# fetty31/fast_LIMO

Hardware: AMD Instinct MI355X
Metric: scans/sec (64k-pt scan, 1M-pt map) + kNN HBM GB/s vs roofline; ATE vs CPU ref (higher is better)
Workload: dtype f32; 1 GPU; BASELINE.json configs[1]: 65536-pt Velodyne-like scan (64 rings x 1024 azimuths), 1000000-pt box-world map, k=5, MAX_NUM_ITERS=3, GPU deskew + iterated ESKF update per step; parallelism=replicas x1 (independent scan streams, no collective), steps_bit_reproducible=True, chains_run=0, chains_handed_back_early=0, chains_declined=2597

## Files before the change

fast_limo_amd/csrc/hip/flimo_kernels.hip:

```cpp
#include <hip/hip_runtime.h>
#include <hip/hip_ext.h>
#include <float.h>
#include <limits.h>
#include <stdlib.h>
#include <algorithm>
#include "flimo_types.h"
#include "flimo_math.h"
#include "flimo_kernels.h"
#include "flimo_chain.h"
#include "flimo_ieskf.h"

#pragma clang fp contract(off)

namespace flimo {

FLIMO_DEV bool pair_less(float d0, int i0, float d1, int i1) { return (d0 < d1) || (d0 == d1 && i0 < i1); }

template <int K>
FLIMO_DEV void topk_insert(float (&bd)[K], int (&bi)[K], float d, int id) {
  if (!pair_less(d, id, bd[K - 1], bi[K - 1])) return;
  bd[K - 1] = d;
  bi[K - 1] = id;
#pragma unroll
  for (int s = K - 1; s > 0; s--) {
// ... 32 lines not shown
FLIMO_DEV void merge_group(float (&bd)[K], int (&bi)[K]) {
#pragma unroll
  for (int off = 1; off < L; off <<= 1) {
    float od[K];
    int oi[K];
#pragma unroll
    for (int s = 0; s < K; s++) {
      od[s] = __shfl_xor(bd[s], off, 64);
      oi[s] = __shfl_xor(bi[s], off, 64);
    }
#pragma unroll
    for (int s = 0; s < K; s++) topk_insert<K>(bd, bi, od[s], oi[s]);
  }
}

FLIMO_DEV float slab_dist(int d, float r) {
  return d == 0 ? 0.f : (d > 0 ? ((float)d - r) : (r + (float)(-d - 1)));
}

template <int K = 5>
struct KnnResultK {
  float bd[K];
  int bi[K];
  int cand;
  bool exact;
};
typedef KnnResultK<5> KnnResult;

template <int L, int K>
FLIMO_DEV void visit_row(const GridView& G, int cx, int cy, int cz, int dy, int dz, int r_prev, int r, float rx,
                         float ry, float rz, float margin, float cell2, float bound, int sub, float gx, float gy,
                         float gz, KnnResultK<K>& R) {
  const float a = fmaxf(slab_dist(dy, ry) - margin, 0.f), b = fmaxf(slab_dist(dz, rz) - margin, 0.f);
  const float yz2 = a * a + b * b;
  if (yz2 * cell2 >= fminf(bound, R.bd[K - 1])) return;
  if (max(abs(dy), abs(dz)) > r_prev) {
    const int x0 = max(cx - r, 0), x1 = min(cx + r, G.nx - 1);
    if (x0 <= x1) {
      uint32_t lo, hi;
      grid_row_range(G, G.dir, cy + dy, cz + dz, x0 * G.xs, (x1 + 1) * G.xs, lo, hi);
      scan_range<L, K>(G.pts, lo, hi, sub, gx, gy, gz, R.bd, R.bi, R.cand);
    }
  } else {
    {
      const int x0 = max(cx - r, 0), x1 = min(cx - r_prev - 1, G.nx - 1);
      const float sx = fmaxf(slab_dist(-(r_prev + 1), rx) - margin, 0.f);
      if (x0 <= x1 && (sx * sx + yz2) * cell2 < fminf(bound, R.bd[K - 1])) {
        uint32_t lo, hi;
        grid_row_range(G, G.dir, cy + dy, cz + dz, x0 * G.xs, (x1 + 1) * G.xs, lo, hi);
        scan_range<L, K>(G.pts, lo, hi, sub, gx, gy, gz, R.bd, R.bi, R.cand);
      }
    }
    {
      const int x0 = max(cx + r_prev + 1, 0), x1 = min(cx + r, G.nx - 1);
      const float sx = fmaxf(slab_dist(r_prev + 1, rx) - margin, 0.f);
      if (x0 <= x1 && (sx * sx + yz2) * cell2 < fminf(bound, R.bd[K - 1])) {
        uint32_t lo, hi;
        grid_row_range(G, G.dir, cy + dy, cz + dz, x0 * G.xs, (x1 + 1) * G.xs, lo, hi);
        scan_range<L, K>(G.pts, lo, hi, sub, gx, gy, gz, R.bd, R.bi, R.cand);
      }
    }
  }
}

template <int L, int K = 5>
FLIMO_DEV void knn_search(const GridView& G, float gx, float gy, float gz, int sub, int max_ring, KnnResultK<K>& R) {
#pragma unroll
  for (int s = 0; s < K; s++) { R.bd[s] = FLT_MAX; R.bi[s] = INT_MAX; }
  R.cand = 0;
  R.exact = false;

  const float fx = (gx - G.ox) * G.inv_cell, fy = (gy - G.oy) * G.inv_cell, fz = (gz - G.oz) * G.inv_cell;
  if (!(fx == fx) || !(fy == fy) || !(fz == fz)) return;
  const float lim = 1.0e9f;
  const float flx = floorf(fminf(fmaxf(fx, -lim), lim));
  const float fly = floorf(fminf(fmaxf(fy, -lim), lim));
  const float flz = floorf(fminf(fmaxf(fz, -lim), lim));
  const int cx = (int)flx - G.six, cy = (int)fly - G.siy, cz = (int)flz - G.siz;
  const float rx = fminf(fmaxf(fx - flx, 0.f), 1.f), ry = fminf(fmaxf(fy - fly, 0.f), 1.f),
              rz = fminf(fmaxf(fz - flz, 0.f), 1.f);

  const int maxdim = grid_maxdim(G);
  const float margin = 1.0e-3f + 4.0e-7f * (float)maxdim;
  const float cell2 = G.cell * G.cell;
  const float edge = fminf(fminf(fminf(rx, 1.f - rx), fminf(ry, 1.f - ry)), fminf(rz, 1.f - rz));

  int r0;
  {
    const int ox_ = cx < 0 ? -cx : (cx >= G.nx ? cx - G.nx + 1 : 0);
    const int oy_ = cy < 0 ? -cy : (cy >= G.ny ? cy - G.ny + 1 : 0);
    const int oz_ = cz < 0 ? -cz : (cz >= G.nz ? cz - G.nz + 1 : 0);
    r0 = max(1, max(ox_, max(oy_, oz_)));
  }
  if (r0 > max_ring) return;

  int r_prev = -1;
  int r = r0;
  float bound = FLT_MAX;
  for (;;) {
    if (r == 1) {
      uint32_t lo[9], hi[9];
      const int x0 = max(cx - 1, 0), x1 = min(cx + 1, G.nx - 1);
#pragma unroll
      for (int t = 0; t < 9; t++) {
        const int dy = (t % 3 == 0) ? 0 : ((t % 3 == 1) ? -1 : 1);
        const int dz = (t / 3 == 0) ? 0 : ((t / 3 == 1) ? -1 : 1);
        const int yy = cy + dy, zz = cz + dz;
        const bool in = (yy >= 0) && (yy < G.ny) && (zz >= 0) && (zz < G.nz) && (x0 <= x1);
        lo[t] = 0u; hi[t] = 0u;
        if (in) grid_row_range(G, G.dir, yy, zz, x0 * G.xs, (x1 + 1) * G.xs, lo[t], hi[t]);
      }
#pragma unroll
      for (int t = 0; t < 9; t++) {
        const int dy = (t % 3 == 0) ? 0 : ((t % 3 == 1) ? -1 : 1);
        const int dz = (t / 3 == 0) ? 0 : ((t / 3 == 1) ? -1 : 1);
        const float a = fmaxf(slab_dist(dy, ry) - margin, 0.f), b = fmaxf(slab_dist(dz, rz) - margin, 0.f);
        if ((a * a + b * b) * cell2 >= R.bd[K - 1]) continue;
        scan_range<L, K>(G.pts, lo[t], hi[t], sub, gx, gy, gz, R.bd, R.bi, R.cand);
      }
    } else {
      const int dz0 = max(-r, -cz), dz1 = min(r, G.nz - 1 - cz);
      const int dy0 = max(-r, -cy), dy1 = min(r, G.ny - 1 - cy);
      for (int dz = dz0; dz <= dz1; dz++)
        for (int dy = dy0; dy <= dy1; dy++)
          visit_row<L, K>(G, cx, cy, cz, dy, dz, r_prev, r, rx, ry, rz, margin, cell2, bound, sub, gx, gy, gz, R);
    }
    if (L > 1) merge_group<L, K>(R.bd, R.bi);
    const float rg = ((float)r + edge - margin) * G.cell;
    const bool have5 = R.bi[K - 1] != INT_MAX;
    const bool covers = (cx - r <= 0) && (cx + r >= G.nx - 1) && (cy - r <= 0) && (cy + r >= G.ny - 1) &&
                        (cz - r <= 0) && (cz + r >= G.nz - 1);
    if (covers || (have5 && R.bd[K - 1] <= rg * rg * (1.f - 1.0e-6f))) { R.exact = true; break; }
    if (r >= max_ring) break;
    int rn = 2 * r;
    if (have5) {
      bound = R.bd[K - 1];
      const float need = fl_sqrt(R.bd[K - 1]) * G.inv_cell * (1.f + 4.0e-6f) - edge + margin;
      rn = max(r + 1, (int)ceilf(fminf(need, 1.0e9f)));
    }
    rn = min(rn, max_ring);
    if (L > 1 && sub != 0) {
#pragma unroll
      for (int s = 0; s < K; s++) { R.bd[s] = FLT_MAX; R.bi[s] = INT_MAX; }
    }
    r_prev = r;
    r = rn;
  }
}

typedef unsigned long long u64;
#define KEY_EMPTY 0xffffffffffffffffull

#ifdef FLIMO_TRACE
__device__ unsigned long long g_trace[2][16384 * 8];
#if FLIMO_TRACE == 2
__shared__ unsigned long long s_trace_lds[2][8];
#define TRACE(k, slot)                                                                                  \
  do {                                                                                                  \
    asm volatile("s_waitcnt vmcnt(0) lgkmcnt(0)" ::: "memory");                                         \
    if (threadIdx.x == 0) s_trace_lds[k][slot] = wall_clock64();                                        \
  } while (0)
#define TRACE_LANE(k, slot, tid)                                                                        \
  do {                                                                                                  \
    if (threadIdx.x == (tid)) {                                                                         \
      asm volatile("s_waitcnt vmcnt(0) lgkmcnt(0)" ::: "memory");                                       \
      s_trace_lds[k][slot] = wall_clock64();                                                            \
    }                                                                                                   \
  } while (0)
#define TRACE_FLUSH()                                                                                   \
  do {                                                                                                  \
    __syncthreads();                                                                                    \
    if (threadIdx.x == 0 && blockIdx.x < 16384)                                                         \
      for (int k_ = 0; k_ < 2; k_++) for (int s_ = 0; s_ < 8; s_++) g_trace[k_][blockIdx.x * 8 + s_] = s_trace_lds[k_][s_]; \
  } while (0)
#else
#define TRACE(k, slot)                                                                                  \
  do {                                                                                                  \
    asm volatile("s_waitcnt vmcnt(0) lgkmcnt(0)" ::: "memory");                                         \
    if (threadIdx.x == 0 && blockIdx.x < 16384) g_trace[k][blockIdx.x * 8 + (slot)] = wall_clock64();  \
  } while (0)
#define TRACE_FLUSH() do {} while (0)
#define TRACE_LANE(k, slot, tid) do {} while (0)
#endif
extern "C" int flimo_trace_read(int k, unsigned long long* out, size_t n) {
  return (int)hipMemcpyFromSymbol(out, HIP_SYMBOL(g_trace), n * sizeof(unsigned long long), (size_t)k * 16384 * 8 * sizeof(unsigned long long),
                                  hipMemcpyDeviceToHost);
}
#else
#define TRACE(k, slot) do {} while (0)
#define TRACE_FLUSH() do {} while (0)
#define TRACE_LANE(k, slot, tid) do {} while (0)
#endif

FLIMO_DEV u64 make_key(float d, uint32_t idx) { return ((u64)__float_as_uint(d) << 32) | (u64)idx; }

FLIMO_DEV void key5_insert(u64 (&k)[5], u64 key) {
  if (key >= k[4]) return;
  k[4] = key;
#pragma unroll
  for (int s = 4; s > 0; s--) {
    const u64 a = k[s - 1], b = k[s];
    const bool sw = b < a;
    k[s - 1] = sw ? b : a;
    k[s] = sw ? a : b;
  }
}

__constant__ int c_stripe = 8;
void set_xcd_stripe(int stripe) { (void)hipMemcpyToSymbol(HIP_SYMBOL(c_stripe), &stripe, sizeof(int)); }

__device__ __forceinline__ int xcd_chunk(int b, int nb) {
  const int x = b & 7, k = b >> 3, per = nb >> 3;
  const int S = c_stripe;
  if (S <= 0 || S >= per) return x * per + k;
  const int full = (per / S) * S;
  if (k >= full) return 8 * full + x * (per - full) + (k - full);
  return ((k / S) * 8 + x) * S + (k % S);
}

struct NbrRec {
  int32_t idx[5];
  int32_t flag;
  int32_t d5_bits;
  int32_t d5_valid;
};

struct U3 { uint32_t a, b, c; };
struct __attribute__((aligned(8))) Seg2 { uint32_t x0, y0, x1, y1; };
__device__ __forceinline__ double key_min(double a, double b) { double r; asm("v_min_f64 %0, %1, %2" : "=v"(r) : "v"(a), "v"(b)); return r; }
__device__ __forceinline__ double key_max(double a, double b) { double r; asm("v_max_f64 %0, %1, %2" : "=v"(r) : "v"(a), "v"(b)); return r; }
__device__ __forceinline__ double key_make(float d, uint32_t id) { return __hiloint2double((int)__float_as_uint(d), (int)id); }
__device__ __forceinline__ void best5_insert(double (&k)[5], double x) {
  double t = x;
#pragma unroll
  for (int i = 0; i < 4; i++) {
    const double lo = key_min(k[i], t);
    t = key_max(k[i], t);
    k[i] = lo;
  }
  k[4] = key_min(k[4], t);
}
__device__ __forceinline__ void best6_insert(double (&k)[6], double x) {
  double t = x;
#pragma unroll
  for (int i = 0; i < 5; i++) {
    const double lo = key_min(k[i], t);
    t = key_max(k[i], t);
    k[i] = lo;
  }
  k[5] = key_min(k[5], t);
}
#define KEY_NONE 0x7f800000ffffffffull

template <int CTRL>
__device__ __forceinline__ double key_dpp(double x) {
  const int lo = __double2loint(x), hi = __double2hiint(x);
  const int l2 = __builtin_amdgcn_update_dpp(lo, lo, CTRL, 0xf, 0xf, false);
  const int h2 = __builtin_amdgcn_update_dpp(hi, hi, CTRL, 0xf, 0xf, false);
  return __hiloint2double(h2, l2);
}
__device__ __forceinline__ double key_group_min(double md, int Gl, int lane) {
  md = key_min(md, key_dpp<0xB1>(md));
  if (Gl >= 4) md = key_min(md, key_dpp<0x4E>(md));
  if (Gl >= 8) md = key_min(md, key_dpp<0x141>(md));
  if (Gl >= 16) md = key_min(md, key_dpp<0x140>(md));
  if (Gl >= 32) {
    const int lo = __double2loint(md), hi = __double2hiint(md);
    const double r0 = __hiloint2double(__builtin_amdgcn_readlane(hi, 0), __builtin_amdgcn_readlane(lo, 0));
    const double r1 = __hiloint2double(__builtin_amdgcn_readlane(hi, 16), __builtin_amdgcn_readlane(lo, 16));
    const double r2 = __hiloint2double(__builtin_amdgcn_readlane(hi, 32), __builtin_amdgcn_readlane(lo, 32));
    const double r3 = __hiloint2double(__builtin_amdgcn_readlane(hi, 48), __builtin_amdgcn_readlane(lo, 48));
    const double a = key_min(r0, r1), b = key_min(r2, r3);
    md = (Gl >= 64) ? key_min(a, b) : (lane < 32 ? a : b);
  }
  return md;
}

__device__ __forceinline__ void key_merge6(const double (&a)[6], const double (&b)[6], double (&c)[6]) {
#pragma unroll
  for (int i = 0; i < 6; i++) c[i] = key_min(a[i], b[5 - i]);
#define FLIMO_CE(i, j) { const double lo_ = key_min(c[i], c[j]); c[j] = key_max(c[i], c[j]); c[i] = lo_; }
  FLIMO_CE(0, 5) FLIMO_CE(1, 3) FLIMO_CE(2, 4)
  FLIMO_CE(1, 2) FLIMO_CE(3, 4)
  FLIMO_CE(0, 3) FLIMO_CE(2, 5)
  FLIMO_CE(0, 1) FLIMO_CE(2, 3) FLIMO_CE(4, 5)
  FLIMO_CE(1, 2) FLIMO_CE(3, 4)
#undef FLIMO_CE
}
__device__ __forceinline__ void key_pair_merge6(const double (&a)[6], double (&c)[6]) {
  double b[6];
#pragma unroll
  for (int i = 0; i < 6; i++) b[i] = key_dpp<0xB1>(a[i]);
  key_merge6(a, b, c);
}

template <int L, int N, bool PAYW = false, int NSEG = 9>
__device__ __forceinline__ void knn5_body(const float4* __restrict__ pts, uint32_t s0, uint32_t total, uint32_t last,
                                          const uint32_t (&off)[NSEG + 1], const uint32_t (&dl)[NSEG], float gx, float gy, float gz,
                                          double (&k5)[6]) {
  float4 pt[N];
  uint32_t id[N];
#pragma unroll
  for (int u = 0; u < N; u++) {
    const uint32_t s = min(s0 + u * L, last);
    uint32_t delta = dl[0];
#pragma unroll
    for (int t = 1; t < NSEG; t++) delta = (s >= off[t]) ? dl[t] : delta;
    id[u] = s + delta;
    pt[u] = pts[id[u]];
  }
  if constexpr (N == 8)
    asm volatile("" : "+v"(pt[0].x), "+v"(pt[0].y), "+v"(pt[0].z), "+v"(pt[1].x), "+v"(pt[1].y), "+v"(pt[1].z),
                      "+v"(pt[2].x), "+v"(pt[2].y), "+v"(pt[2].z), "+v"(pt[3].x), "+v"(pt[3].y), "+v"(pt[3].z),
                      "+v"(pt[4].x), "+v"(pt[4].y), "+v"(pt[4].z), "+v"(pt[5].x), "+v"(pt[5].y), "+v"(pt[5].z),
                      "+v"(pt[6].x), "+v"(pt[6].y), "+v"(pt[6].z), "+v"(pt[7].x), "+v"(pt[7].y), "+v"(pt[7].z));
  else if constexpr (N == 4)
    asm volatile("" : "+v"(pt[0].x), "+v"(pt[0].y), "+v"(pt[0].z), "+v"(pt[1].x), "+v"(pt[1].y), "+v"(pt[1].z),
                      "+v"(pt[2].x), "+v"(pt[2].y), "+v"(pt[2].z), "+v"(pt[3].x), "+v"(pt[3].y), "+v"(pt[3].z));
  else if constexpr (N == 2)
    asm volatile("" : "+v"(pt[0].x), "+v"(pt[0].y), "+v"(pt[0].z), "+v"(pt[1].x), "+v"(pt[1].y), "+v"(pt[1].z));
#pragma unroll
  for (int u = 0; u < N; u++) {
    const bool live = s0 + u * L < total;
    const float d = sqdist3(gx, gy, gz, pt[u].x, pt[u].y, pt[u].z);
    best6_insert(k5, key_make(live ? d : INFINITY, live ? (PAYW ? __float_as_uint(pt[u].w) : id[u]) : 0xffffffffu));
  }
}


struct FitIdx { unsigned char raw[FIT_LIVE_PAD]; };
__device__ __forceinline__ bool key_has_tie(const u64 (&best)[5], u64 sixth) {
  const uint32_t d0 = (uint32_t)(best[0] >> 32), d1 = (uint32_t)(best[1] >> 32), d2 = (uint32_t)(best[2] >> 32),
                 d3 = (uint32_t)(best[3] >> 32), d4 = (uint32_t)(best[4] >> 32), d5 = (uint32_t)(sixth >> 32);
  return (d0 == d1) | (d1 == d2) | (d2 == d3) | (d3 == d4) | (d4 == d5);
}
constexpr int TAIL_MAX_RING = 3;
constexpr int KNN_FAR_RING = 4;
constexpr uint32_t PROBE_MIN_OWN = 6;
struct __align__(16) WaveLds {
  float tile[16 * 65];
  double acc[256];
  int src[64];
  int res[64][8];
};
// ... 758 lines not shown
    if (in_range && sub == 0 && flag == 1 && inside) {
      int4 a, b;
      a.x = (int)(uint32_t)best[0]; a.y = (int)(uint32_t)best[1]; a.z = (int)(uint32_t)best[2]; a.w = (int)(uint32_t)best[3];
      b.x = (int)(uint32_t)best[4]; b.y = 4; b.z = (int)(uint32_t)(best[4] >> 32);
      b.w = (int)(1u | (tie ? 2u : 0u) | ((uint32_t)(fa.seq & 0xffffffull) << 8));
      int4* o = reinterpret_cast<int4*>(&nbr[p]);
      o[0] = a;
      o[1] = b;
      if (tie && tl.list) { const unsigned slot = atomicAdd(tl.count, 1u); if (slot < tl.cap) tl.list[slot] = p; }
    }
    return;
  }
  TRACE(0, 4);
  const bool pend_tail = tail && in_range && flag == 2;
  if (in_range && sub == 0 && !pend_tail) {
    int4 a, b;
    a.x = (int)(uint32_t)best[0]; a.y = (int)(uint32_t)best[1]; a.z = (int)(uint32_t)best[2]; a.w = (int)(uint32_t)best[3];
    b.x = (int)(uint32_t)best[4]; b.y = min(flag, 2); b.z = (int)(uint32_t)(best[4] >> 32); b.w = ((flag == 1) ? 1 : 0) | (tie ? 2 : 0);
    if (tie && !tie_listed && tl.list) { const unsigned slot = atomicAdd(tl.count, 1u); if (slot < tl.cap) tl.list[slot] = p; }
    int4* o = reinterpret_cast<int4*>(&nbr[p]);
    o[0] = a;
    o[1] = b;
    if (flag >= 2) {
      const int slot = atomicAdd(wl_count, 1);
      int4* e = reinterpret_cast<int4*>(wl) + 2 * (size_t)slot;
      e[0] = make_int4(p, __float_as_int(gx), __float_as_int(gy), __float_as_int(gz));
      e[1] = make_int4((int)(uint32_t)(best[4] >> 32), 2, __float_as_int(b2), 0);
    }
  }
  WaveLds& W = s_w[threadIdx.x >> 6];
  if (tail) knn5_tail(G, dir, max_ring, nbr, pend_tail && sub == 0, p, gx, gy, gz, (uint32_t)(best[4] >> 32), b2, W, wl_count, cand_total, FUSE, tl);
  TRACE(0, 5);
  if constexpr (FUSE) {
    const int lane = threadIdx.x & 63;
    float v[16];
#pragma unroll
    for (int i = 0; i < 16; i++) v[i] = 0.f;
    wave_lds_sync();
    int ids[5] = {(int)(uint32_t)best[0], (int)(uint32_t)best[1], (int)(uint32_t)best[2], (int)(uint32_t)best[3], (int)(uint32_t)best[4]};
    int fl = flag;
    bool tied = tie;
    uint32_t d5b = (uint32_t)(best[4] >> 32);
    if (sub == 0 && in_range && pend_tail) {
      const int4* rr = reinterpret_cast<const int4*>(W.res[lane]);
      const int4 a = rr[0], b = rr[1];
      ids[0] = a.x; ids[1] = a.y; ids[2] = a.z; ids[3] = a.w; ids[4] = b.x;
      fl = b.y;
      tied = (b.w & 2) != 0;
      d5b = (uint32_t)b.z;
    }
    if (fa.book.node_c)
      tie_repair_wave(G, fa.book, nbr, sub == 0 && in_range && fl == 1 && tied, p, gx, gy, gz, d5b, ids, *reinterpret_cast<TieLds*>(W.tile));
    TRACE(1, 1);
    if (sub == 0 && in_range) {
      if (fl == 1 && __float_as_uint(sp.w) < (uint32_t)fa.mp.n_queries) fit_row(G, P, fa.mp, ids, gx, gy, gz, v);
    }
    TRACE(1, 3);
    wave_lds_sync();
    fit_reduce_publish<64 / L>(v, sub == 0, lane / L, W.tile, s_w[0].acc, s_w[1].acc, s_w[2].acc, s_w[3].acc, &s_last, fa.idx,
                               fa.partials, fa.granules, fa.ticket, wl_count, fa.seq, tl, (int)blockIdx.x, nb);
  }
  TRACE_FLUSH();
}

template <int L, int SLOTS, bool FUSE, bool FINE = false>
__global__ __launch_bounds__(256) KNN_WPE void knn5_kernel(GridView G, const float4* __restrict__ scan_sorted, int n,
                                                   PoseMats P, int max_ring, NbrRec* __restrict__ nbr,
                                                   int* __restrict__ wl, int* __restrict__ wl_count,
                                                   unsigned long long* __restrict__ cand_total, PrevPass prev, int tail,
                                                   FuseArgs fa) {
  __shared__ __align__(16) uint16_t s_dir[GRID_DIR_MAX];
  const DirRegs dr = grid_dir_fetch(G);
  __shared__ PoseMats s_pose;
  static_assert(sizeof(PoseMats) % 4 == 0 && sizeof(PoseMats) / 4 <= 256, "one word per thread");
  if (threadIdx.x < sizeof(PoseMats) / 4)
    reinterpret_cast<uint32_t*>(&s_pose)[threadIdx.x] = reinterpret_cast<const uint32_t*>(&P)[threadIdx.x];
  knn5_pass<L, SLOTS, FUSE, FINE>(G, s_dir, &dr, scan_sorted, n, s_pose, max_ring, nbr, wl, wl_count, cand_total, prev.RT, prev.valid, prev.probe_min, tail, fa);
}
__device__ __forceinline__ const ChainHead* chain_enter(const ChainHead* __restrict__ H, const PipeHead* __restrict__ pipe, const PrevRT& prt,
                                                        unsigned int wait_epoch, unsigned int end_code) {
  constexpr int NW = (int)(sizeof(ChainHead) / 4);
  __shared__ unsigned int s_head[NW];
  __shared__ int s_go;
  if (pipe != nullptr) {
    const int tid = (int)threadIdx.x;
    if (tid < 64) {
      const unsigned long long t0 = wall_clock64();
      int go = 0;
      unsigned long long gv = 0ull;
      unsigned int* dec = const_cast<unsigned int*>(&pipe->decision);
      const unsigned int v_go = wait_epoch, v_pend = wait_epoch | 0x80000000u, v_no = (wait_epoch & 0x3fffffffu) | 0x80000000u;
      for (int look = 0;; look++) {
        const unsigned int d = __hip_atomic_load(dec, __ATOMIC_RELAXED, __HIP_MEMORY_SCOPE_SYSTEM);
        gv = __hip_atomic_load(&pipe->gran[tid], __ATOMIC_RELAXED, __HIP_MEMORY_SCOPE_SYSTEM);
        const unsigned int e = (unsigned int)(gv >> 32);
        const bool all = __ballot(e == wait_epoch) == ~0ull;
        const unsigned int e0 = (unsigned int)__builtin_amdgcn_readfirstlane((int)e);
        if (d == v_no) break;
        if (d == v_pend) { __builtin_amdgcn_s_sleep(8); continue; }
        if (all) { go = 1; break; }
        if (e0 == end_code) break;
        const unsigned long long waited = wall_clock64() - t0;
        if (blockIdx.x == 0 && d != v_go && waited > (unsigned long long)CH_POLL_MS * 100000ull) {
          if (tid == 0) __hip_atomic_store(dec, v_pend, __ATOMIC_RELAXED, __HIP_MEMORY_SCOPE_SYSTEM);
          asm volatile("s_waitcnt vmcnt(0)" ::: "memory");
          for (int nap = 0; nap < 4; nap++) __builtin_amdgcn_s_sleep(127);
          gv = __hip_atomic_load(&pipe->gran[tid], __ATOMIC_RELAXED, __HIP_MEMORY_SCOPE_SYSTEM);
          go = __ballot((unsigned int)(gv >> 32) == wait_epoch) == ~0ull ? 1 : 0;
          if (tid == 0) __hip_atomic_store(dec, go ? v_go : v_no, __ATOMIC_RELAXED, __HIP_MEMORY_SCOPE_SYSTEM);
          break;
        }
        if (waited > 4ull * (unsigned long long)CH_POLL_MS * 100000ull) break;
        if (look == 0) __builtin_amdgcn_s_sleep(48);
        else __builtin_amdgcn_s_sleep(8);
      }
      if (go && tid < PH_WORDS) s_head[tid < 36 ? (tid / 12) * 16 + tid % 12 : tid + 12] = (unsigned int)gv;
      if (tid == 0) s_go = go;
    } else if (tid < 64 + 12) {
      const int k = tid - 64;
      s_head[(k / 4) * 16 + 12 + k % 4] = __float_as_uint(k % 4 == 3 ? 1.f : 0.f);
    } else if (tid >= 128 && tid < 128 + 16) {
      s_head[offsetof(ChainHead, prev_RT) / 4 + (tid - 128)] = __float_as_uint(prt.v[tid - 128]);
    } else if (tid >= 192 && tid < 192 + NW - (int)(offsetof(ChainHead, status) / 4)) {
      s_head[offsetof(ChainHead, status) / 4 + (tid - 192)] = 0u;
    }
    __syncthreads();
    if (!s_go) return nullptr;
  } else {
    if ((int)threadIdx.x < NW) s_head[threadIdx.x] = reinterpret_cast<const unsigned int*>(H)[threadIdx.x];
    __syncthreads();
  }
  const ChainHead* Lh = reinterpret_cast<const ChainHead*>(s_head);
  return Lh->status != 0 ? nullptr : Lh;
}
template <int L, int SLOTS, bool FUSE, bool FINE = false>
__global__ __launch_bounds__(256) KNN_WPE void knn5_chain_kernel(GridView G, const float4* __restrict__ scan_sorted, int n,
                                                   const ChainHead* __restrict__ H, int max_ring, NbrRec* __restrict__ nbr,
                                                   int* __restrict__ wl, int* __restrict__ wl_count,
                                                   unsigned long long* __restrict__ cand_total, int prev_valid, unsigned probe_min, int tail,
                                                   FuseArgs fa, unsigned int wait_epoch, const PipeHead* __restrict__ pipe, PrevRT prt) {
  __shared__ __align__(16) uint16_t s_dir[GRID_DIR_MAX];
  {
    const DirRegs dr = grid_dir_fetch(G);
    grid_dir_store(s_dir, dr);
  }
  const ChainHead* Lh = chain_enter(H, pipe, prt, wait_epoch, fa.ch.end_code);
  if (!Lh) return;
  knn5_pass<L, SLOTS, FUSE, FINE>(G, s_dir, nullptr, scan_sorted, n, Lh->pose, max_ring, nbr, wl, wl_count, cand_total, Lh->prev_RT, prev_valid, probe_min, tail, fa);
}

__device__ __forceinline__ void widen_body(const GridView& G, int max_ring, NbrRec* __restrict__ nbr,
                                           const int* __restrict__ wl, const int* __restrict__ wl_count,
                                           unsigned long long* __restrict__ cand_total, int first_ring, const TieList& tl,
                                           int blk, int nblk, uint32_t (*s_off)[65], uint32_t (*s_lo)[64]) {
  const int lane = threadIdx.x & 63, wave = threadIdx.x >> 6;
  const int maxdim = grid_maxdim(G);
  const float margin = 1.0e-3f + 4.0e-7f * (float)maxdim;
  int w = blk * 4 + wave;
  const int4* entries = reinterpret_cast<const int4*>(wl);
  int4 e0 = entries[2 * (size_t)w], e1 = entries[2 * (size_t)w + 1];
  const int count = *wl_count;
  for (; w < count; w += nblk * 4) {
    if (w != blk * 4 + wave) { e0 = entries[2 * (size_t)w]; e1 = entries[2 * (size_t)w + 1]; }
    const int p = e0.x;
    const float gx = __int_as_float(e0.y), gy = __int_as_float(e0.z), gz = __int_as_float(e0.w);
    const int hint_bits = e1.x;
    const float fx = (gx - G.ox) * G.inv_cell, fy = (gy - G.oy) * G.inv_cell, fz = (gz - G.oz) * G.inv_cell;
    const float flx = floorf(fminf(fmaxf(fx, -1.0e9f), 1.0e9f)), fly = floorf(fminf(fmaxf(fy, -1.0e9f), 1.0e9f)),
                flz = floorf(fminf(fmaxf(fz, -1.0e9f), 1.0e9f));
    const int cx = (int)flx - G.six, cy = (int)fly - G.siy, cz = (int)flz - G.siz;
    const float rx = fminf(fmaxf(fx - flx, 0.f), 1.f), ry = fminf(fmaxf(fy - fly, 0.f), 1.f),
                rz = fminf(fmaxf(fz - flz, 0.f), 1.f);
    const float edge = fminf(fminf(fminf(rx, 1.f - rx), fminf(ry, 1.f - ry)), fminf(rz, 1.f - rz));
    u64 best[5] = {KEY_NONE, KEY_NONE, KEY_NONE, KEY_NONE, KEY_NONE};
    u64 sixth = KEY_NONE;
    int flag = 0;
    int cand = 0;
    int r = first_ring;
    float bnd2 = __int_as_float(e1.z);
    if (!(bnd2 >= 0.f)) bnd2 = INFINITY;
    {
      const float hint = __int_as_float(hint_bits);
      if (hint >= 0.f && hint < INFINITY) {
        const float need = fl_sqrt(hint) * G.inv_cell * (1.f + 4.0e-6f) - edge + margin;
        r = max(2, (int)ceilf(fminf(need, 1.0e9f)));
        const float rc = (fl_sqrt(hint) * (1.f + 1.0e-5f) + 1.0e-6f) * G.inv_cell;
        bnd2 = fminf(bnd2, rc * rc * (1.f + 1.0e-5f));
      }
      r = min(r, max_ring);
    }
    for (;;) {
      const int side = 2 * r + 1;
      uint32_t lo = 0, len = 0;
      if (lane < side * side) {
        const int dy = (lane % side) - r, dz = (lane / side) - r;
        const int yy = cy + dy, zz = cz + dz;
        const float a_ = fmaxf(slab_dist(dy, ry) - margin, 0.f), b_ = fmaxf(slab_dist(dz, rz) - margin, 0.f);
        const float dyz2 = a_ * a_ + b_ * b_;
        int x0 = max(cx - r, 0), x1 = min(cx + r, G.nx - 1);
        if (bnd2 < 1.0e18f) {
          const float xr = fl_sqrt(fmaxf(bnd2 - dyz2, 0.f)) * (1.f + 1.0e-6f) + margin + 1.0e-4f;
          const int dr = (int)fminf(floorf(fminf(xr + rx, 1.0e6f)), (float)r);
          const int dl = (int)fminf(floorf(fminf(xr + (1.f - rx), 1.0e6f)), (float)r);
          x0 = max(cx - dl, 0); x1 = min(cx + dr, G.nx - 1);
        }
        if (dyz2 <= bnd2 && yy >= 0 && yy < G.ny && zz >= 0 && zz < G.nz && x0 <= x1) {
          uint32_t hi_;
          grid_row_range(G, G.dir, yy, zz, x0 * G.xs, (x1 + 1) * G.xs, lo, hi_);
          len = hi_ - lo;
        }
      }
      uint32_t inc = len;
#pragma unroll
      for (int o = 1; o < 64; o <<= 1) {
        const uint32_t v = __shfl_up(inc, o, 64);
        if (lane >= o) inc += v;
      }
      const uint32_t total = __shfl(inc, 63, 64);
      s_off[wave][lane + 1] = inc;
      if (lane == 0) s_off[wave][0] = 0;
      s_lo[wave][lane] = lo;
      __builtin_amdgcn_wave_barrier();
      const double none = __longlong_as_double((long long)KEY_NONE);
      double k5[6] = {none, none, none, none, none, none};
      const uint32_t last = total - 1u;
      for (uint32_t s0 = (uint32_t)lane; s0 < total; s0 += 4 * 64) {
        float4 q[4];
        uint32_t id[4];
#pragma unroll
        for (int u = 0; u < 4; u++) {
          const uint32_t s = min(s0 + 64u * u, last);
          int a = 0;
#pragma unroll
          for (int step = 32; step >= 1; step >>= 1) a = (s_off[wave][a + step] <= s) ? a + step : a;
          id[u] = s_lo[wave][a] + (s - s_off[wave][a]);
          q[u] = G.pts[id[u]];
        }
        asm volatile("" : "+v"(q[0].x), "+v"(q[0].y), "+v"(q[0].z), "+v"(q[1].x), "+v"(q[1].y), "+v"(q[1].z),
                          "+v"(q[2].x), "+v"(q[2].y), "+v"(q[2].z), "+v"(q[3].x), "+v"(q[3].y), "+v"(q[3].z));
#pragma unroll
        for (int u = 0; u < 4; u++) {
          const bool live = s0 + 64u * u < total;
          const float d = sqdist3(gx, gy, gz, q[u].x, q[u].y, q[u].z);
          best6_insert(k5, key_make(live ? d : INFINITY, live ? id[u] : 0xffffffffu));
        }
      }
      cand += total > (uint32_t)lane ? (int)((total - (uint32_t)lane + 63u) / 64u) : 0;
      __builtin_amdgcn_wave_barrier();
      u64 mine[6];
#pragma unroll
      for (int i = 0; i < 6; i++) mine[i] = (u64)__double_as_longlong(k5[i]);
#pragma unroll
      for (int k = 0; k < 6; k++) {
        const double md = key_group_min(__longlong_as_double((long long)mine[0]), 64, lane);
        const u64 m = (u64)__double_as_longlong(md);
        if (k < 5) best[k] = m; else sixth = m;
        if (mine[0] == m) { mine[0] = mine[1]; mine[1] = mine[2]; mine[2] = mine[3]; mine[3] = mine[4]; mine[4] = mine[5]; mine[5] = KEY_NONE; }
      }
      const float rg = ((float)r + edge - margin) * G.cell;
      const float d5 = __uint_as_float((uint32_t)(best[4] >> 32));
      const bool have5 = d5 < INFINITY;
      const bool covers = (cx - r <= 0) && (cx + r >= G.nx - 1) && (cy - r <= 0) && (cy + r >= G.ny - 1) &&
                          (cz - r <= 0) && (cz + r >= G.nz - 1);
      if (have5 && (covers || d5 <= rg * rg * (1.f - 1.0e-6f))) { flag = 1; break; }
      if (covers || r >= max_ring) { flag = 0; break; }
      int rn = r + 1;
      if (have5) {
        const float need = fl_sqrt(d5) * G.inv_cell * (1.f + 4.0e-6f) - edge + margin;
        rn = max(r + 1, (int)ceilf(fminf(need, 1.0e9f)));
        const float rc = (fl_sqrt(d5) * (1.f + 1.0e-5f) + 1.0e-6f) * G.inv_cell;
        bnd2 = fminf(bnd2, rc * rc * (1.f + 1.0e-5f));
      }
      r = min(rn, max_ring);
    }
    if (cand_total) {
      int c = cand;
#pragma unroll
      for (int o = 1; o < 64; o <<= 1) c += __shfl_xor(c, o, 64);
      if (lane == 0) atomicAdd(cand_total, (unsigned long long)c);
    }
    if (lane == 0) {
      int4 a, b;
      a.x = (int)(uint32_t)best[0]; a.y = (int)(uint32_t)best[1]; a.z = (int)(uint32_t)best[2]; a.w = (int)(uint32_t)best[3];
      const bool tie = flag == 1 && key_has_tie(best, sixth);
      b.x = (int)(uint32_t)best[4]; b.y = flag; b.z = (int)(uint32_t)(best[4] >> 32); b.w = ((flag == 1) ? 1 : 0) | (tie ? 2 : 0);
      int4* o = reinterpret_cast<int4*>(&nbr[p]);
      o[0] = a;
      o[1] = b;
      if (tie && tl.list) { const unsigned slot = atomicAdd(tl.count, 1u); if (slot < tl.cap) tl.list[slot] = p; }
    }
  }
}
__global__ __launch_bounds__(256) void widen_kernel(GridView G, const float4* __restrict__ scan_sorted, PoseMats P,
                                                    int max_ring, NbrRec* __restrict__ nbr, const int* __restrict__ wl,
                                                    const int* __restrict__ wl_count,
                                                    unsigned long long* __restrict__ cand_total, int first_ring, TieList tl,
                                                    const ChainHead* __restrict__ H) {
  __shared__ uint32_t s_off[4][65];
  __shared__ uint32_t s_lo[4][64];
  if (H && H->status != 0) return;
  widen_body(G, max_ring, nbr, wl, wl_count, cand_total, first_ring, tl, (int)blockIdx.x, (int)gridDim.x, s_off, s_lo);
}

__global__ __launch_bounds__(256) void widen_general_kernel(GridView G, const float4* __restrict__ scan_sorted,
                                                            PoseMats P, int max_ring, NbrRec* __restrict__ nbr,
                                                            const int* __restrict__ wl, const int* __restrict__ wl_count, TieList tl) {
  constexpr int L = 16;
  const int count = *wl_count;
  const int sub = threadIdx.x % L;
  for (int w = blockIdx.x * (256 / L) + threadIdx.x / L; w < count; w += gridDim.x * (256 / L)) {
    const int p = reinterpret_cast<const int4*>(wl)[2 * (size_t)w].x;
    const float4 sp = scan_sorted[p];
    float gx, gy, gz;
    xform4(P.RT, sp.x, sp.y, sp.z, gx, gy, gz);
    KnnResult R;
    knn_search<L>(G, gx, gy, gz, sub, max_ring, R);
    if (sub == 0) {
      const bool ok = R.exact && (R.bi[4] != INT_MAX);
      int4 a, b;
      a.x = R.bi[0]; a.y = R.bi[1]; a.z = R.bi[2]; a.w = R.bi[3];
      b.x = R.bi[4]; b.y = ok ? 1 : 0; b.z = ok ? __float_as_int(R.bd[4]) : 0; b.w = ok ? 3 : 0;
      int4* o = reinterpret_cast<int4*>(&nbr[p]);
      o[0] = a;
      o[1] = b;
      if (ok && tl.list) { const unsigned slot = atomicAdd(tl.count, 1u); if (slot < tl.cap) tl.list[slot] = p; }
    }
  }
}

typedef double double4_t __attribute__((ext_vector_type(4)));


template <bool RECS, bool DBG, int FIT_THREADS>
__global__ __launch_bounds__(FIT_THREADS) void fit_kernel(GridView G, const float4* __restrict__ scan_sorted, int n,
                                                          const NbrRec* __restrict__ nbr, PoseMats P, MatchParams mp,
                                                          double* __restrict__ partials, Rec16* __restrict__ recs,
                                                          RecDbg* __restrict__ dbg, double* __restrict__ out256,
                                                          unsigned int* __restrict__ ticket, int* __restrict__ wl_count,
                                                          unsigned long long seq) {
  constexpr int FIT_WAVES = FIT_THREADS / 64;
  __shared__ float s_rec[FIT_WAVES][16 * 65];
  __shared__ double s_acc[FIT_WAVES][256];
  __shared__ unsigned int s_last;
  const int chunk = xcd_chunk(blockIdx.x, gridDim.x);
  const int p = chunk * FIT_THREADS + threadIdx.x;
  const int lane = threadIdx.x & 63, wave = threadIdx.x >> 6;

  float v[16];
#pragma unroll
  for (int i = 0; i < 16; i++) v[i] = 0.f;
  float n4[4] = {0.f, 0.f, 0.f, 0.f};
  float gx = 0.f, gy = 0.f, gz = 0.f;
  float sq[5] = {0.f, 0.f, 0.f, 0.f, 0.f};
  int ids[5] = {-1, -1, -1, -1, -1};
  int flag = 0;
  uint32_t orig = 0;
  bool valid = false;
  TRACE(1, 0);
  if (p < n) {
    const float4 sp = scan_sorted[p];
    orig = __float_as_uint(sp.w);
    xform4(P.RT, sp.x, sp.y, sp.z, gx, gy, gz);
    const int4* nb = reinterpret_cast<const int4*>(&nbr[p]);
    const int4 a = nb[0], b = nb[1];
    ids[0] = a.x; ids[1] = a.y; ids[2] = a.z; ids[3] = a.w; ids[4] = b.x;
    flag = b.y;
    valid = (flag == 1) && (orig < (uint32_t)mp.n_queries);
    TRACE(1, 1);
    if (valid) {
      float px[5], py[5], pz[5];
#pragma unroll
      for (int s = 0; s < 5; s++) {
        const float4 q = G.pts[ids[s]];
        px[s] = q.x; py[s] = q.y; pz[s] = q.z;
        sq[s] = sqdist3(gx, gy, gz, q.x, q.y, q.z);
      }
      TRACE(1, 2);
      valid = (double)sq[4] < mp.max_dist_plane_d;
      if (valid) {
        plane_fit5(px, py, pz, n4);
        valid = plane_eval5(n4, px, py, pz, mp.plane_threshold);
      }
      if (valid) {
        const float dist = n4[0] * gx + n4[1] * gy + n4[2] * gz + n4[3];
        float row[12];
        h_row(P, gx, gy, gz, n4, mp.estimate_extrinsics, row);
#pragma unroll
        for (int i = 0; i < 12; i++) v[i] = row[i];
        v[12] = -dist;
        v[13] = 1.f;
      }
    }
    if (RECS && orig < (uint32_t)mp.n_queries) {
      float4* out = reinterpret_cast<float4*>(&recs[orig]);
      out[0] = make_float4(v[0], v[1], v[2], v[3]);
      out[1] = make_float4(v[4], v[5], v[6], v[7]);
      out[2] = make_float4(v[8], v[9], v[10], v[11]);
      out[3] = make_float4(v[12], v[13], 0.f, 0.f);
      if (DBG) {
        RecDbg d;
#pragma unroll
        for (int i = 0; i < 4; i++) d.n[i] = valid ? n4[i] : 0.f;
        d.p_global[0] = gx; d.p_global[1] = gy; d.p_global[2] = gz;
        int cnt = 0;
#pragma unroll
        for (int s = 0; s < 5; s++) {
          const bool has = (flag == 1);
          cnt += has ? 1 : 0;
          d.sqd[s] = has ? sq[s] : 0.f;
          d.nbr[s] = has ? (int32_t)__float_as_uint(G.pts[ids[s]].w) : -1;
        }
        d.n_nbr = cnt;
        d.cand = 0;
        d.pad = 0;
        dbg[orig] = d;
      }
    }
  }
  TRACE(1, 3);
  if (partials == nullptr) return;
  float* sr = s_rec[wave];
#pragma unroll
  for (int c = 0; c < 16; c++) sr[c * 65 + lane] = v[c];
  __builtin_amdgcn_wave_barrier();
  __syncthreads();
  double4_t acc = {0.0, 0.0, 0.0, 0.0};
  const int col = lane & 15, sub4 = lane >> 4;
#pragma unroll
  for (int s = 0; s < 16; s++) {
    const double a = (double)sr[col * 65 + 4 * s + sub4];
    acc = __builtin_amdgcn_mfma_f64_16x16x4f64(a, a, acc, 0, 0, 0);
  }
  double* sa = s_acc[wave];
  sa[lane * 4 + 0] = acc[0]; sa[lane * 4 + 1] = acc[1]; sa[lane * 4 + 2] = acc[2]; sa[lane * 4 + 3] = acc[3];
  __syncthreads();
  if (threadIdx.x < 256) {
    const int t = threadIdx.x;
    double r = 0.0;
#pragma unroll
    for (int w = 0; w < FIT_WAVES; w++) r += s_acc[w][t];
    __hip_atomic_store(&partials[(size_t)blockIdx.x * 256 + t], r, __ATOMIC_RELAXED, __HIP_MEMORY_SCOPE_AGENT);
  }
  asm volatile("s_waitcnt vmcnt(0)" ::: "memory");
  __syncthreads();
  TRACE(1, 4);
  const int group = blockIdx.x & (FIT_GROUPS - 1);
  const int nb_g = (int)(gridDim.x / FIT_GROUPS);
  if (threadIdx.x == 0) {
    const unsigned int old = __hip_atomic_fetch_add(ticket + group, 1u, __ATOMIC_RELAXED, __HIP_MEMORY_SCOPE_AGENT);
    s_last = (old == (unsigned int)nb_g - 1u) ? 1u : 0u;
  }
  __syncthreads();
  TRACE(1, 5);
  if (s_last) {
// ... 1101 lines not shown
```

Baseline: 7918 scans/s.

## Scalarize widen-kernel per-wave state and stage grid directory in LDS

Forces the per-wave work-list entry fields, cell coordinates, ring radius and bound into scalar registers with readfirstlane, so the ring loop runs on uniform SGPR state instead of VGPRs. Grid directory lookups are served from a shared-memory copy loaded at kernel start, and its fetch is issued together with the first work-list loads, before the chain status check. The per-wave candidate count reduction is replaced by the uniform total, using readlane instead of a shuffle. Trace-only instrumentation for the widen pass is also added. The costs are extra LDS per block and a directory fetch even when the chain status exits early; the candidate statistic now counts total candidates rather than per-lane iterations.

```diff
diff --git a/fast_limo_amd/csrc/hip/flimo_kernels.hip b/fast_limo_amd/csrc/hip/flimo_kernels.hip
--- a/fast_limo_amd/csrc/hip/flimo_kernels.hip
+++ b/fast_limo_amd/csrc/hip/flimo_kernels.hip
@@ -208,7 +208,7 @@
 #define KEY_EMPTY 0xffffffffffffffffull
 
 #ifdef FLIMO_TRACE
-__device__ unsigned long long g_trace[2][16384 * 8];
+__device__ unsigned long long g_trace[3][16384 * 8];
 #if FLIMO_TRACE == 2
 __shared__ unsigned long long s_trace_lds[2][8];
 #define TRACE(k, slot)                                                                                  \
@@ -229,6 +229,12 @@
     if (threadIdx.x == 0 && blockIdx.x < 16384)                                                         \
       for (int k_ = 0; k_ < 2; k_++) for (int s_ = 0; s_ < 8; s_++) g_trace[k_][blockIdx.x * 8 + s_] = s_trace_lds[k_][s_]; \
   } while (0)
+__shared__ unsigned long long s_trace_widen[8];
+#define TRACE_WIDEN(slot)                                                                               \
+  do {                                                                                                  \
+    asm volatile("s_waitcnt vmcnt(0) lgkmcnt(0)" ::: "memory");                                         \
+    if (threadIdx.x == 0) s_trace_widen[slot] = wall_clock64();                                         \
+  } while (0)
 #else
 #define TRACE(k, slot)                                                                                  \
   do {                                                                                                  \
@@ -246,6 +252,9 @@
 #define TRACE(k, slot) do {} while (0)
 #define TRACE_FLUSH() do {} while (0)
 #define TRACE_LANE(k, slot, tid) do {} while (0)
+#endif
+#ifndef TRACE_WIDEN
+#define TRACE_WIDEN(slot) do {} while (0)
 #endif
 
 FLIMO_DEV u64 make_key(float d, uint32_t idx) { return ((u64)__float_as_uint(d) << 32) | (u64)idx; }
@@ -1310,32 +1319,49 @@
 __device__ __forceinline__ void widen_body(const GridView& G, int max_ring, NbrRec* __restrict__ nbr,
                                            const int* __restrict__ wl, const int* __restrict__ wl_count,
                                            unsigned long long* __restrict__ cand_total, int first_ring, const TieList& tl,
-                                           int blk, int nblk, uint32_t (*s_off)[65], uint32_t (*s_lo)[64]) {
-  const int lane = threadIdx.x & 63, wave = threadIdx.x >> 6;
+                                           int blk, int nblk, uint32_t (*s_off)[65], uint32_t (*s_lo)[64], uint16_t* s_dir,
+                                           const ChainHead* __restrict__ H) {
+  const auto uni_i = [](int v) { return __builtin_amdgcn_readfirstlane(v); };
+  const auto uni_f = [](float v) { return __int_as_float(__builtin_amdgcn_readfirstlane(__float_as_int(v))); };
+  const int lane = threadIdx.x & 63, wave = uni_i((int)(threadIdx.x >> 6));
   const int maxdim = grid_maxdim(G);
   const float margin = 1.0e-3f + 4.0e-7f * (float)maxdim;
   int w = blk * 4 + wave;
+#if defined(FLIMO_TRACE) && FLIMO_TRACE == 2
+  const unsigned long long t_start = wall_clock64();
+#endif
   const int4* entries = reinterpret_cast<const int4*>(wl);
+  const DirRegs dr = grid_dir_fetch(G);
   int4 e0 = entries[2 * (size_t)w], e1 = entries[2 * (size_t)w + 1];
   const int count = *wl_count;
+  if (H && H->status != 0) return;
+  grid_dir_store(s_dir, dr);
+#if defined(FLIMO_TRACE) && FLIMO_TRACE == 2
+  if (threadIdx.x == 0) for (int s_ = 0; s_ < 8; s_++) s_trace_widen[s_] = 0ull;
+  TRACE_WIDEN(1);
+  if (threadIdx.x == 0) s_trace_widen[0] = t_start;
+#endif
   for (; w < count; w += nblk * 4) {
     if (w != blk * 4 + wave) { e0 = entries[2 * (size_t)w]; e1 = entries[2 * (size_t)w + 1]; }
-    const int p = e0.x;
-    const float gx = __int_as_float(e0.y), gy = __int_as_float(e0.z), gz = __int_as_float(e0.w);
-    const int hint_bits = e1.x;
+#if defined(FLIMO_TRACE) && FLIMO_TRACE == 2
+    const bool stamped = w == blk * 4 + wave;
+#endif
+    const int p = uni_i(e0.x);
+    const float gx = __int_as_float(uni_i(e0.y)), gy = __int_as_float(uni_i(e0.z)), gz = __int_as_float(uni_i(e0.w));
+    const int hint_bits = uni_i(e1.x);
     const float fx = (gx - G.ox) * G.inv_cell, fy = (gy - G.oy) * G.inv_cell, fz = (gz - G.oz) * G.inv_cell;
     const float flx = floorf(fminf(fmaxf(fx, -1.0e9f), 1.0e9f)), fly = floorf(fminf(fmaxf(fy, -1.0e9f), 1.0e9f)),
                 flz = floorf(fminf(fmaxf(fz, -1.0e9f), 1.0e9f));
-    const int cx = (int)flx - G.six, cy = (int)fly - G.siy, cz = (int)flz - G.siz;
-    const float rx = fminf(fmaxf(fx - flx, 0.f), 1.f), ry = fminf(fmaxf(fy - fly, 0.f), 1.f),
-                rz = fminf(fmaxf(fz - flz, 0.f), 1.f);
-    const float edge = fminf(fminf(fminf(rx, 1.f - rx), fminf(ry, 1.f - ry)), fminf(rz, 1.f - rz));
+    const int cx = uni_i((int)flx - G.six), cy = uni_i((int)fly - G.siy), cz = uni_i((int)flz - G.siz);
+    const float rx = uni_f(fminf(fmaxf(fx - flx, 0.f), 1.f)), ry = uni_f(fminf(fmaxf(fy - fly, 0.f), 1.f)),
+                rz = uni_f(fminf(fmaxf(fz - flz, 0.f), 1.f));
+    const float edge = uni_f(fminf(fminf(fminf(rx, 1.f - rx), fminf(ry, 1.f - ry)), fminf(rz, 1.f - rz)));
     u64 best[5] = {KEY_NONE, KEY_NONE, KEY_NONE, KEY_NONE, KEY_NONE};
     u64 sixth = KEY_NONE;
     int flag = 0;
     int cand = 0;
     int r = first_ring;
-    float bnd2 = __int_as_float(e1.z);
+    float bnd2 = __int_as_float(uni_i(e1.z));
     if (!(bnd2 >= 0.f)) bnd2 = INFINITY;
     {
       const float hint = __int_as_float(hint_bits);
@@ -1345,7 +1371,8 @@
         const float rc = (fl_sqrt(hint) * (1.f + 1.0e-5f) + 1.0e-6f) * G.inv_cell;
         bnd2 = fminf(bnd2, rc * rc * (1.f + 1.0e-5f));
       }
-      r = min(r, max_ring);
+      r = uni_i(min(r, max_ring));
+      bnd2 = uni_f(bnd2);
     }
     for (;;) {
       const int side = 2 * r + 1;
@@ -1364,17 +1391,20 @@
         }
         if (dyz2 <= bnd2 && yy >= 0 && yy < G.ny && zz >= 0 && zz < G.nz && x0 <= x1) {
           uint32_t hi_;
-          grid_row_range(G, G.dir, yy, zz, x0 * G.xs, (x1 + 1) * G.xs, lo, hi_);
+          grid_row_range(G, s_dir, yy, zz, x0 * G.xs, (x1 + 1) * G.xs, lo, hi_);
           len = hi_ - lo;
         }
       }
+#if defined(FLIMO_TRACE) && FLIMO_TRACE == 2
+      if (stamped) { TRACE_WIDEN(2); if (threadIdx.x == 0) s_trace_widen[6] += 1ull; }
+#endif
       uint32_t inc = len;
 #pragma unroll
       for (int o = 1; o < 64; o <<= 1) {
         const uint32_t v = __shfl_up(inc, o, 64);
         if (lane >= o) inc += v;
       }
-      const uint32_t total = __shfl(inc, 63, 64);
+      const uint32_t total = (uint32_t)__builtin_amdgcn_readlane((int)inc, 63);
       s_off[wave][lane + 1] = inc;
       if (lane == 0) s_off[wave][0] = 0;
       s_lo[wave][lane] = lo;
@@ -1403,8 +1433,11 @@
           best6_insert(k5, key_make(live ? d : INFINITY, live ? id[u] : 0xffffffffu));
         }
       }
-      cand += total > (uint32_t)lane ? (int)((total - (uint32_t)lane + 63u) / 64u) : 0;
+      cand += (int)total;
       __builtin_amdgcn_wave_barrier();
+#if defined(FLIMO_TRACE) && FLIMO_TRACE == 2
+      if (stamped) { TRACE_WIDEN(3); if (threadIdx.x == 0) s_trace_widen[7] += (unsigned long long)total; }
+#endif
       u64 mine[6];
 #pragma unroll
       for (int i = 0; i < 6; i++) mine[i] = (u64)__double_as_longlong(k5[i]);
@@ -1415,6 +1448,9 @@
         if (k < 5) best[k] = m; else sixth = m;
         if (mine[0] == m) { mine[0] = mine[1]; mine[1] = mine[2]; mine[2] = mine[3]; mine[3] = mine[4]; mine[4] = mine[5]; mine[5] = KEY_NONE; }
       }
+#if defined(FLIMO_TRACE) && FLIMO_TRACE == 2
+      if (stamped) TRACE_WIDEN(4);
+#endif
       const float rg = ((float)r + edge - margin) * G.cell;
       const float d5 = __uint_as_float((uint32_t)(best[4] >> 32));
       const bool have5 = d5 < INFINITY;
@@ -1427,16 +1463,11 @@
         const float need = fl_sqrt(d5) * G.inv_cell * (1.f + 4.0e-6f) - edge + margin;
         rn = max(r + 1, (int)ceilf(fminf(need, 1.0e9f)));
         const float rc = (fl_sqrt(d5) * (1.f + 1.0e-5f) + 1.0e-6f) * G.inv_cell;
-        bnd2 = fminf(bnd2, rc * rc * (1.f + 1.0e-5f));
-      }
-      r = min(rn, max_ring);
-    }
-    if (cand_total) {
-      int c = cand;
-#pragma unroll
-      for (int o = 1; o < 64; o <<= 1) c += __shfl_xor(c, o, 64);
-      if (lane == 0) atomicAdd(cand_total, (unsigned long long)c);
-    }
+        bnd2 = uni_f(fminf(bnd2, rc * rc * (1.f + 1.0e-5f)));
+      }
+      r = uni_i(min(rn, max_ring));
+    }
+    if (cand_total && lane == 0) atomicAdd(cand_total, (unsigned long long)cand);
     if (lane == 0) {
       int4 a, b;
       a.x = (int)(uint32_t)best[0]; a.y = (int)(uint32_t)best[1]; a.z = (int)(uint32_t)best[2]; a.w = (int)(uint32_t)best[3];
@@ -1447,7 +1478,13 @@
       o[1] = b;
       if (tie && tl.list) { const unsigned slot = atomicAdd(tl.count, 1u); if (slot < tl.cap) tl.list[slot] = p; }
     }
-  }
+#if defined(FLIMO_TRACE) && FLIMO_TRACE == 2
+    if (stamped) TRACE_WIDEN(5);
+#endif
+  }
+#if defined(FLIMO_TRACE) && FLIMO_TRACE == 2
+  if (threadIdx.x == 0) for (int s_ = 0; s_ < 8; s_++) g_trace[2][blk * 8 + s_] = s_trace_widen[s_];
+#endif
 }
 __global__ __launch_bounds__(256) void widen_kernel(GridView G, const float4* __restrict__ scan_sorted, PoseMats P,
                                                     int max_ring, NbrRec* __restrict__ nbr, const int* __restrict__ wl,
@@ -1456,8 +1493,8 @@
                                                     const ChainHead* __restrict__ H) {
   __shared__ uint32_t s_off[4][65];
   __shared__ uint32_t s_lo[4][64];
-  if (H && H->status != 0) return;
-  widen_body(G, max_ring, nbr, wl, wl_count, cand_total, first_ring, tl, (int)blockIdx.x, (int)gridDim.x, s_off, s_lo);
+  __shared__ __align__(16) uint16_t s_dir[GRID_DIR_MAX];
+  widen_body(G, max_ring, nbr, wl, wl_count, cand_total, first_ring, tl, (int)blockIdx.x, (int)gridDim.x, s_off, s_lo, s_dir, H);
 }
 
 __global__ __launch_bounds__(256) void widen_general_kernel(GridView G, const float4* __restrict__ scan_sorted,
```

New measurement: 7941 scans/s, median of 2. About the same (+0.3%).
